# nirschl-lab/stain2stain

Hardware: AMD Instinct MI355X
Metric: paired 256x256 stain tiles/sec (full CFM optimisation step) (higher is better)
Workload: dtype bf16

## Files before the change

### include/stain2stain_hip.h

```cpp
#ifndef STAIN2STAIN_HIP_H
#define STAIN2STAIN_HIP_H

#ifdef __cplusplus
extern "C" {
#endif

#define S2S_OK 0
#define S2S_ERR_SHAPE (-1)
#define S2S_ERR_ALIGN (-2)
#define S2S_ERR_DTYPE (-3)
#define S2S_ERR_LAUNCH (-4)
#define S2S_ERR_NULL (-5)

#define S2S_BF16 0
#define S2S_F32 1

int s2s_conv3x3_stat_blocks(int dtype, int B, int H, int W, int Cout);
int s2s_conv3x3_nhwc(int dtype, const void* x0, int ld0, int c0, const void* x1, int ld1, int c1,
                     const void* w_packed, const float* bias, void* y, int ldy, float* stat_part,
                     const float* ep_scale, const float* ep_shift, int relu, int B, int H, int W, int Cout,
                     void* stream);

int s2s_conv3x3_ksplit(int dtype, int B, int H, int W, int Cout, int cin);
int s2s_conv3x3_nhwc_k(int dtype, const void* x0, int ld0, int c0, const void* x1, int ld1, int c1,
                       const void* w_packed, const float* bias, void* y, int ldy, float* stat_part,
                       const float* ep_scale, const float* ep_shift, int relu, float* kwork, int B, int H, int W,
                       int Cout, void* stream);
int s2s_conv3x3_stat_rows(int dtype, int B, int H, int W, int Cout, int c0, int c1, int ld0, int ld1, int has_bias);
int s2s_conv3x3_staged(int dtype, int B, int H, int W, int Cout, int c0, int c1, int ld0, int ld1, int ldy, int stats);
int s2s_conv3x3_family(int dtype, int B, int H, int W, int Cout, int c0, int c1, int ld0, int ld1, int ldy, int has_bias,
                       int has_affine, int stats, int stat_rows, int kwork);
int s2s_conv3x3_nhwc_s(int dtype, const void* x0, int ld0, int c0, const void* x1, int ld1, int c1, const void* w_packed,
                       const float* bias, void* y, int ldy, float* stat_part, int stat_rows, const float* ep_scale,
                       const float* ep_shift, int relu, float* kwork, int B, int H, int W, int Cout, void* stream);
int s2s_debug_conv_clock(long* out_host, int n);

int s2s_conv3x3_wgrad_splits(int dtype, int B, int H, int W, int Cin, int Cout);
int s2s_conv3x3_wgrad_nhwc(int dtype, const void* dy, int lddy, int Cout, const void* x0, int ld0, int c0,
                           const void* x1, int ld1, int c1, float* part, float* grad_oihw, int accumulate,
                           int B, int H, int W, void* stream);
int s2s_conv3x3_wgrad_phase(int dtype, const void* dy, int lddy, int Cout, const void* x0, int ld0, int c0,
                            const void* x1, int ld1, int c1, float* part, float* grad_oihw, int accumulate,
                            int B, int H, int W, int phases, void* stream);

int s2s_stem_stat_blocks(int B, int H, int W);
int s2s_stem_conv3x3_fwd(int dtype, const float* x_nchw, const float* w_oihw, const float* bias, void* y, int ldy,
                         float* stat_part, int B, int H, int W, int Cin, int Cout, void* stream);
int s2s_stem_wgrad_blocks(int B, int H, int W);
int s2s_stem_conv3x3_wgrad(int dtype, const void* dy, int lddy, const float* x_nchw, float* part, float* dw_oihw,
                           float* dbias, int accumulate, int B, int H, int W, int Cin, int Cout, void* stream);
int s2s_head_conv1x1_fwd(int dtype, const void* x, int ldx, const float* w, const float* bias, float* y_nchw, int B,
                         int H, int W, int C, int Cout, void* stream);
int s2s_head_wgrad_blocks(int B, int H, int W);
int s2s_head_conv1x1_bwd(int dtype, const float* dy_nchw, const void* x, int ldx, const float* w, void* dx, int lddx,
                         float* part, float* dw, float* dbias, int accumulate, int B, int H, int W, int C, int Cout,
                         void* stream);

int s2s_head_loss_blocks(int B, int H, int W);
int s2s_head_loss_fused(int dtype, const void* x, int ldx, const float* w, const float* bias, const float* u_nchw,
                        float* v_nchw, void* dx, int lddx, float grad_scale, float* part, double* lpart, float* dw,
                        float* dbias, float* loss, int accumulate, int B, int H, int W, int C, int Cout, void* stream);

int s2s_tail_blocks(int B, int H, int W);
int s2s_tail_fwd_loss(int dtype, const void* raw, int ldx, const float* scale, const float* shift, const float* mean,
                      const float* invstd, const float* w, const float* bias, const float* u_nchw, float* v_nchw,
                      float* g_nchw, float grad_scale, float* part, double* lpart, float* bnwork, float* dw,
                      float* dbias, float* loss, float* dgamma, float* dbeta, float* conv_dbias, int accumulate, int B,
                      int H, int W, int C, int Cout, void* stream);
int s2s_tail_bwd_apply(int dtype, const void* raw, int ldx, const float* g_nchw, const float* w, const float* scale,
                       const float* shift, const float* mean, const float* invstd, const float* gamma,
                       const float* bnwork, void* dx, int lddx, int B, int H, int W, int C, int Cout, void* stream);

int s2s_bn_finalize(const float* part, int nblk, int C, long count, const float* gamma, const float* beta,
                    float* running_mean, float* running_var, long* num_batches_tracked, float momentum, float eps,
                    float* mean, float* invstd, float* scale, float* shift, void* stream);
int s2s_bn_finalize_b(const float* part, int nblk, int C, long count, const float* gamma, const float* beta,
                      float* running_mean, float* running_var, long* num_batches_tracked, float momentum, float eps,
                      float* mean, float* invstd, float* scale, float* shift, const float* conv_bias, void* stream);
int s2s_bn_eval_prepare(int C, const float* gamma, const float* beta, const float* running_mean,
                        const float* running_var, float eps, float* scale, float* shift, void* stream);
int s2s_bn_relu_apply(int dtype, const void* x, int ldx, const float* scale, const float* shift, void* y, int ldy,
                      void* pool, int ldp, int B, int H, int W, int C, void* stream);
int s2s_maxpool2(int dtype, const void* x, int ldx, void* pool, int ldp, int B, int H, int W, int C, void* stream);
int s2s_bn_bwd_blocks(int B, int H, int W, int C);
int s2s_bn_relu_bwd(int dtype, const void* g1, int ldg1, const void* gp, int ldgp, const float* scale,
                    const float* shift, const void* x, int ldx, const float* mean, const float* invstd, const float* gamma, float* dgamma,
                    float* dbeta, float* dbias_conv, int accumulate, void* dx, int lddx, float* work, int B, int H,
                    int W, int C, void* stream);
int s2s_bn_partial_sums(const float* part, int nblk, int C, float* sums, void* stream);
int s2s_bn_relu_bwd_phase(int dtype, const void* g1, int ldg1, const void* gp, int ldgp, const float* scale,
                          const float* shift, const void* x, int ldx, const float* mean, const float* invstd,
                          const float* gamma, float* dgamma, float* dbeta, float* dbias_conv, int accumulate, void* dx,
                          int lddx, float* work, int B, int H, int W, int C, long count_total, int phases, void* stream);

int s2s_upsample2x_bilinear_ac_fwd(int dtype, const void* x, int ldx, const float* bias_nc, void* y, int ldy, int B,
                                   int Hin, int Win, int Hout, int Wout, int C, void* stream);
int s2s_upsample2x_bilinear_ac_bwd(int dtype, const void* dy, int lddy, void* dx, int lddx, int B, int Hin, int Win,
                                   int Hout, int Wout, int C, void* stream);
int s2s_upsample2x_bilinear_ac_bwd_ref(int dtype, const void* dy, int lddy, void* dx, int lddx, int B, int Hin,
                                       int Win, int Hout, int Wout, int C, void* stream);
int s2s_upsample2x_bwd_family(int lddy, int lddx, int B, int Hin, int Win, int Hout, int Wout, int C, int reference);
int s2s_pixel_sum(int dtype, const void* x, int ldx, float* out_nc, int B, int HW, int C, int accumulate,
                  void* stream);

int s2s_time_embedding(const float* t, float* out, int B, int dim, void* stream);
int s2s_linear_fwd(const float* x, const float* w, const float* bias, float* y, int B, int K, int N, void* stream);
int s2s_linear_bwd(const float* dy, const float* x, const float* w, float* dx, float* dw, float* db, int accumulate,
                   int B, int K, int N, void* stream);
int s2s_silu_fwd(const float* h, float* a, int n, void* stream);
int s2s_silu_bwd(const float* h, const float* da, float* dh, int n, void* stream);
int s2s_cfm_sample(const float* x0, const float* x1, const float* t, const float* eps, float sigma, float* xt,
                   float* ut, int B, long per_sample, void* stream);
int s2s_mse_loss(const float* v, const float* u, float* dv, float grad_scale, float* loss, double* work, long count,
                 void* stream);
int s2s_ode_error_norm(const float* e, const float* y0, const float* y1, float atol, float rtol, float* out,
                       double* work, long n, void* stream);
int s2s_axpy(float* x, const float* y, float a, long n, void* stream);
int s2s_dp_partials(long n);
int s2s_dp_init(int phase, const float* y, const float* k1, const float* fa, double* state, double* part, float* out,
                float* t_out, int* status, float atol, float rtol, int B, long n, void* stream);
int s2s_dp_stage(int i, const float* y, const float* k1, const float* k2, const float* k3, const float* k4,
                 const float* k5, const float* k6, const double* state, float* out, float* t_out, int B, long n,
                 void* stream);
int s2s_dp_error(const float* k1, const float* k2, const float* k3, const float* k4, const float* k5, const float* k6,
                 const float* k7, const float* y, const float* y_new, const double* state, double* part, float atol,
                 float rtol, int B, long n, void* stream);
int s2s_dp_control(double* state, const double* part, int* status, int max_steps, int B, long n, void* stream);
int s2s_dp_commit(float* y, const float* y_new, float* k1, const float* k7, const double* state, int B, long n,
                  void* stream);
int s2s_rk_stage(const float* x, const float* k1, const float* k2, const float* k3, float c1, float c2, float c3, int nk,
                 float* out, float* t_out, const float* table, const int* counter, int stages, int stage, int table_len,
                 int B, long n, void* stream);
int s2s_rk_combine(float* x, const float* k1, const float* k2, const float* k3, const float* k4, float c1, float c2,
                   float c3, float c4, int nk, int* counter, int B, long n, void* stream);
int s2s_fill_f32(float* x, float v, long n, void* stream);
int s2s_euler_tick(float* t, int n, const float* table, int* counter, void* stream);

int s2s_adam_step(float* p, const float* g, float* m, float* v, long n, int step, float lr, float beta1, float beta2,
                  float eps, float weight_decay, float grad_scale, void* stream);
int s2s_adam_step_dev(float* p, const float* g, float* m, float* v, long n, const float* hyper, void* stream);
long s2s_adam_multi_blocks(long n);
int s2s_adam_multi(const void* desc, int ntensors, long total, int step, float lr, float beta1, float beta2, float eps,
                   float weight_decay, float grad_scale, void* stream);
int s2s_adam_ema_step(float* p, const float* g, float* m, float* v, float* ema, long n, int step, float lr, float beta1,
                      float beta2, float eps, float weight_decay, float grad_scale, float ema_weight, void* stream);
int s2s_adam_ema_step_dev(float* p, const float* g, float* m, float* v, float* ema, long n, const float* hyper,
                          const float* ema_weight, void* stream);
long s2s_ema_multi_blocks(long n);
int s2s_ema_multi(const void* desc, int ntensors, long total, const float* weight, void* stream);
long s2s_pack_conv3x3_fwd_elems(int Cout, int Cin);
long s2s_pack_conv3x3_dgrad_elems(int Cout, int Cin);
int s2s_pack_conv3x3(int dtype, const float* w_oihw, void* w_fwd, void* w_dgrad, int Cout, int Cin, void* stream);
int s2s_pack_conv3x3_batched(int dtype, const void* desc, int nlayers, long total, void* stream);
int s2s_nchw_to_nhwc(int dtype, const float* x_nchw, void* y, int ldy, int B, int C, int H, int W, void* stream);
int s2s_nhwc_to_nchw(int dtype, const void* x, int ldx, float* y_nchw, int accumulate, int B, int C, int H, int W,
                     void* stream);

int s2s_paired_crop_flip_normalize(const void* src_u8, const void* tgt_u8, const int* params, float* out_src,
                                   float* out_tgt, int B, int Hs, int Ws, int S, void* stream);
int s2s_pil_resize_bilinear_normalize(const void* src_u8, void* tmp_u8, const int* bounds_h, const int* kk_h,
                                      int ksize_h, const int* bounds_v, const int* kk_v, int ksize_v, void* out_u8,
                                      float* out_f, int B, int Hs, int Ws, int Ho, int Wo, void* stream);

int s2s_region_gather(const void* img_u8, long pitch, int H, int W, int band_top, int band_h, const int* origins,
                      float* out, int B, int T, void* stream);
int s2s_region_blend(const float* tiles, int c0, const float* tiles1, int c1, const int* origins, int n, int T,
                     int overlap, float* acc, int band_rows, int H, int W, int r0, int r1, void* stream);
int s2s_region_finalize(float* acc, int band_rows, int W, int C, int r0, int r1, void* out_u8, long pitch_u8,
                        float* out_f, long pitch_f, int out_top, void* stream);

int s2s_region_tissue_count(const void* img_u8, long pitch, int H, int W, int band_top, int band_h, const int* origins,
                            int n, int T, int white, int black, int* counts, void* stream);
int s2s_region_skip_weight(const int* origins, int n, int T, int overlap, float* ws, int band_rows, int H, int W,
                           int r0, int r1, void* stream);
int s2s_region_finalize_mixed(float* acc, float* ws, int band_rows, int W, int C, int r0, int r1, const void* src_u8,
                              long src_pitch, int src_top, void* out_u8, long pitch_u8, float* out_f, long pitch_f,
                              int out_top, void* stream);

int s2s_seg_loss(const float* z, const float* g, float* dz, float* out, double* work, long n, float smooth,
// ... 175 lines not shown
```

### stain2stain_amd/csrc/resample.hip

```cpp
#include "common.h"
#include <stdlib.h>

namespace {

struct Axis {
  int i0, i1;
  float w0, w1;
};

__device__ __forceinline__ Axis ac_axis(int dst, int n_in, float scale) {
  Axis a;
  const float src = scale * (float)dst;
  a.i0 = (int)src;
  if (a.i0 > n_in - 1) a.i0 = n_in - 1;
  a.i1 = a.i0 + (a.i0 < n_in - 1 ? 1 : 0);
  a.w1 = src - (float)a.i0;
  a.w0 = 1.f - a.w1;
  return a;
}

__device__ __forceinline__ int rs_pcb(int C) {
  int p = 1;
  while (p < 32 && p * 8 < C) p <<= 1;
  return p;
}

template <typename T, bool BIAS>
__global__ __launch_bounds__(256) void upsample2x_fwd_kernel(const T* __restrict__ x, int ldx,
                                                             const float* __restrict__ bias, T* __restrict__ y,
                                                             int ldy, int B, int Hin, int Win, int Hout, int Wout,
                                                             int padT, int padL, int C, int band) {
  const int cp = C >> 3;
  const int Hu = 2 * Hin, Wu = 2 * Win;
  const float sh = Hu > 1 ? (float)(Hin - 1) / (float)(Hu - 1) : 0.f;
  const float sw = Wu > 1 ? (float)(Win - 1) / (float)(Wu - 1) : 0.f;
  const int PCB = rs_pcb(C), WL = 256 / PCB;
  const int pc = threadIdx.x & (PCB - 1), slot = threadIdx.x / PCB;
  const int nrows = B * Hout;
  for (int row0 = blockIdx.x * band; row0 < nrows; row0 += gridDim.x * band)
  for (int row = row0; row < row0 + band && row < nrows; ++row) {
    const int n = row / Hout, oy = row - n * Hout;
    const int uy = oy - padT;
    const bool row_in = uy >= 0 && uy < Hu;
    const Axis ay = ac_axis(row_in ? uy : 0, Hin, sh);
    const T* const r0 = x + ((long)n * Hin + ay.i0) * Win * ldx;
    const T* const r1 = x + ((long)n * Hin + ay.i1) * Win * ldx;
    T* const yr = y + (long)row * Wout * ldy;
    for (int pb = 0; pb < cp; pb += PCB) {
      const int c8 = (pb + pc) * 8;
      if (pb + pc >= cp) continue;
      float bv[8];
#pragma unroll
      for (int k = 0; k < 8; ++k) bv[k] = BIAS ? bias[(long)n * C + c8 + k] : 0.f;
      for (int ox = slot; ox < Wout; ox += WL) {
        const int ux = ox - padL;
        f32x8 o;
        if (!row_in || ux < 0 || ux >= Wu) {
#pragma unroll
          for (int k = 0; k < 8; ++k) o.v[k] = 0.f;
        } else {
          const Axis ax = ac_axis(ux, Win, sw);
          const int o0 = ax.i0 * ldx + c8, o1 = ax.i1 * ldx + c8;
          const f32x8 v00 = load8(r0 + o0), v01 = load8(r0 + o1), v10 = load8(r1 + o0), v11 = load8(r1 + o1);
#pragma unroll
          for (int k = 0; k < 8; ++k) {
            const float b = bv[k];
            o.v[k] = ay.w0 * (ax.w0 * (v00.v[k] + b) + ax.w1 * (v01.v[k] + b)) +
                     ay.w1 * (ax.w0 * (v10.v[k] + b) + ax.w1 * (v11.v[k] + b));
          }
        }
        store8(yr + ox * ldy + c8, o);
      }
    }
  }
}

template <typename T>
__global__ void upsample2x_bwd_kernel(const T* __restrict__ dy, int lddy, T* __restrict__ dx, int lddx, int B,
                                      int Hin, int Win, int Hout, int Wout, int padT, int padL, int C) {
  const int cp = C >> 3;
  const int Hu = 2 * Hin, Wu = 2 * Win;
  const float sh = Hu > 1 ? (float)(Hin - 1) / (float)(Hu - 1) : 0.f;
  const float sw = Wu > 1 ? (float)(Win - 1) / (float)(Wu - 1) : 0.f;
  const int total = B * Hin * Win * cp;
  for (int i = blockIdx.x * blockDim.x + threadIdx.x; i < total; i += gridDim.x * blockDim.x) {
    const int t0 = i / cp, c8 = (i - t0 * cp) * 8;
    const int t1 = t0 / Win, ix = t0 - t1 * Win;
    const int n = t1 / Hin, iy = t1 - n * Hin;
    int y_lo, y_hi, x_lo, x_hi;
    if (Hin == 1) { y_lo = 0; y_hi = Hu - 1; }
    else {
      y_lo = (int)floorf((float)(iy - 1) / sh) - 1; y_hi = (int)ceilf((float)(iy + 1) / sh) + 1;
      if (y_lo < 0) y_lo = 0;
      if (y_hi > Hu - 1) y_hi = Hu - 1;
    }
    if (Win == 1) { x_lo = 0; x_hi = Wu - 1; }
    else {
      x_lo = (int)floorf((float)(ix - 1) / sw) - 1; x_hi = (int)ceilf((float)(ix + 1) / sw) + 1;
      if (x_lo < 0) x_lo = 0;
      if (x_hi > Wu - 1) x_hi = Wu - 1;
    }
    constexpr int NSLOT = 12;
    float wxs[NSLOT];
#pragma unroll
    for (int j = 0; j < NSLOT; ++j) {
      const int ux = x_lo + j;
      float wx = 0.f;
      if (ux <= x_hi) {
        const Axis ax = ac_axis(ux, Win, sw);
        if (ax.i0 == ix) wx += ax.w0;
        if (ax.i1 == ix) wx += ax.w1;
        const int ox = ux + padL;
        if (ox < 0 || ox >= Wout) wx = 0.f;
      }
      wxs[j] = wx;
    }
    f32x8 acc;
#pragma unroll
    for (int k = 0; k < 8; ++k) acc.v[k] = 0.f;
    for (int uy = y_lo; uy <= y_hi; ++uy) {
      const Axis ay = ac_axis(uy, Hin, sh);
      float wy = 0.f;
      if (ay.i0 == iy) wy += ay.w0;
      if (ay.i1 == iy) wy += ay.w1;
      const int oy = uy + padT;
      if (wy == 0.f || oy < 0 || oy >= Hout) continue;
      const T* const rowp = dy + (((long)n * Hout + oy) * Wout + x_lo + padL) * lddy + c8;
#pragma unroll
      for (int j = 0; j < NSLOT; ++j) {
        if (wxs[j] == 0.f) continue;
        const f32x8 g = load8(rowp + (long)j * lddy);
        const float w = wy * wxs[j];
#pragma unroll
        for (int k = 0; k < 8; ++k) acc.v[k] += w * g.v[k];
      }
    }
    store8(dx + (((long)n * Hin + iy) * Win + ix) * lddx + c8, acc);
  }
}

__device__ __forceinline__ float ac_weight_of(int dst, int n_in, float scale, int src_index) {
  const Axis a = ac_axis(dst, n_in, scale);
  return (a.i0 == src_index ? a.w0 : 0.f) + (a.i1 == src_index ? a.w1 : 0.f);
}

template <typename T>
__global__ void upsample2x_bwd_win_kernel(const T* __restrict__ dy, int lddy, T* __restrict__ dx, int lddx, int B,
                                          int Hin, int Win, int Hout, int Wout, int padT, int padL, int C) {
  const int cp = C >> 3;
  const int Hu = 2 * Hin, Wu = 2 * Win;
  const float sh = (float)(Hin - 1) / (float)(Hu - 1), sw = (float)(Win - 1) / (float)(Wu - 1);
  const int total = B * Hin * Win * cp;
  for (int i = blockIdx.x * blockDim.x + threadIdx.x; i < total; i += gridDim.x * blockDim.x) {
    const int t0 = i / cp, c8 = (i - t0 * cp) * 8;
// ... 122 lines not shown
      Raw8<T> cur[6];
#pragma unroll
      for (int m = 0; m < 6; ++m) cur[m] = load_raw8(rowp[j] + off[m]);
      f32x8 g[6];
#pragma unroll
      for (int m = 0; m < 6; ++m) g[m] = widen8(cur[m]);
      if (j < 4) {
#pragma unroll
        for (int m = 0; m < 4; ++m) {
          const float w = wyA[j] * wxA[m];
#pragma unroll
          for (int k = 0; k < 8; ++k) a00.v[k] = fmaf(w, g[m].v[k], a00.v[k]);
        }
#pragma unroll
        for (int m = 0; m < 4; ++m) {
          const float w = wyA[j] * wxB[m];
#pragma unroll
          for (int k = 0; k < 8; ++k) a01.v[k] = fmaf(w, g[m + 2].v[k], a01.v[k]);
        }
      }
      if (j >= 2) {
#pragma unroll
        for (int m = 0; m < 4; ++m) {
          const float w = wyB[j - 2] * wxA[m];
#pragma unroll
          for (int k = 0; k < 8; ++k) a10.v[k] = fmaf(w, g[m].v[k], a10.v[k]);
        }
#pragma unroll
        for (int m = 0; m < 4; ++m) {
          const float w = wyB[j - 2] * wxB[m];
#pragma unroll
          for (int k = 0; k < 8; ++k) a11.v[k] = fmaf(w, g[m + 2].v[k], a11.v[k]);
        }
      }
      if (j < 4) { pin8(a00); pin8(a01); }
      if (j >= 2) { pin8(a10); pin8(a11); }
      __builtin_amdgcn_sched_barrier(0);
    }
    store8(dr0 + ix0 * lddx, a00);
    store8(dr0 + (ix0 + 1) * lddx, a01);
    store8(dr1 + ix0 * lddx, a10);
    store8(dr1 + (ix0 + 1) * lddx, a11);
  }
}

template <typename T>
__global__ void pixel_sum_kernel(const T* __restrict__ x, int ldx, float* __restrict__ out, int HW, int C,
                                 int accumulate) {
  const int n = blockIdx.y;
  const int c = blockIdx.x * 64 + (threadIdx.x & 63);
  const int rg = threadIdx.x >> 6;
  float s = 0.f;
  if (c < C) {
    constexpr int U = 16;
    const T* const xp = x + (long)n * HW * ldx + c;
    int p = rg;
    for (; p + 4 * (U - 1) < HW; p += 4 * U) {
      float v[U];
#pragma unroll
      for (int u = 0; u < U; ++u) v[u] = to_f32(xp[(long)(p + 4 * u) * ldx]);
#pragma unroll
      for (int u = 0; u < U; ++u) s += v[u];
    }
    for (; p < HW; p += 4) s += to_f32(xp[(long)p * ldx]);
  }
  __shared__ float red[4][64];
  red[rg][threadIdx.x & 63] = s;
  __syncthreads();
  if (rg == 0 && c < C) {
    s = red[0][threadIdx.x] + red[1][threadIdx.x] + red[2][threadIdx.x] + red[3][threadIdx.x];
    out[(long)n * C + c] = accumulate ? out[(long)n * C + c] + s : s;
  }
}

inline int ew_grid(long total) {
  long b = (total + 255) / 256;
  if (b > 8192) b = 8192;
  if (b < 1) b = 1;
  return (int)b;
}

}

extern "C" int s2s_upsample2x_bilinear_ac_fwd(int dtype, const void* x, int ldx, const float* bias_nc, void* y,
                                              int ldy, int B, int Hin, int Win, int Hout, int Wout, int C,
                                              void* stream) {
  if (!x || !y) return S2S_ERR_NULL;
  if (B <= 0 || Hin <= 0 || Win <= 0 || C <= 0 || (C % 8) || (ldx % 8) || (ldy % 8)) return S2S_ERR_SHAPE;
  if (Hout < 2 * Hin || Wout < 2 * Win) return S2S_ERR_SHAPE;
  const int padT = (Hout - 2 * Hin) / 2, padL = (Wout - 2 * Win) / 2;
  if ((long)Win * ldx >= (1L << 31) || (long)Wout * ldy >= (1L << 31) || (long)B * Hout >= (1L << 31))
    return S2S_ERR_SHAPE;
  hipStream_t s = (hipStream_t)stream;
  const long rows = (long)B * Hout;
  static const int band_env = [] { const char* e = getenv("S2S_UP_BAND"); return e ? atoi(e) : 0; }();
  const int band = band_env > 0 ? band_env : (rows >= 4096 ? 4 : rows >= 2048 ? 2 : 1);
  const long nwg = (rows + band - 1) / band;
  const dim3 grid((unsigned)(nwg < 65535 * 4 ? nwg : 65535 * 4));
#define S2S_UP(TT, BB)                                                                                          \
  hipLaunchKernelGGL((upsample2x_fwd_kernel<TT, BB>), grid, dim3(256), 0, s, (const TT*)x, ldx, bias_nc, (TT*)y, \
                     ldy, B, Hin, Win, Hout, Wout, padT, padL, C, band)
  if (dtype == S2S_BF16) { if (bias_nc) S2S_UP(bf16_t, true); else S2S_UP(bf16_t, false); }
  else if (dtype == S2S_F32) { if (bias_nc) S2S_UP(float, true); else S2S_UP(float, false); }
  else return S2S_ERR_DTYPE;
#undef S2S_UP
  S2S_LAUNCH_CHECK();
  return S2S_OK;
}

namespace {

enum UpBwdFamily { kUpBwdGather = 0, kUpBwdWindow = 1, kUpBwdQuad = 2 };

int upsample2x_bwd_family(int lddy, int lddx, int B, int Hin, int Win, int Wout, int C, bool reference) {
  if (!(Hin > 3 && Win > 3)) return kUpBwdGather;
  const long nwork = (long)B * ((Hin + 1) / 2);
  const bool quad = !reference && Hin <= 4096 && Win <= 4096 && (long)Wout * lddy < (1L << 31) &&
                    (long)Win * lddx < (1L << 31) && nwork * cdiv(C / 8, 32) < (1L << 31);
  return quad ? kUpBwdQuad : kUpBwdWindow;
}

int upsample2x_bwd_launch(int dtype, const void* dy, int lddy, void* dx, int lddx, int B, int Hin, int Win, int Hout,
                          int Wout, int C, void* stream, bool reference) {
  if (!dy || !dx) return S2S_ERR_NULL;
  if (B <= 0 || Hin <= 0 || Win <= 0 || C <= 0 || (C % 8) || (lddy % 8) || (lddx % 8)) return S2S_ERR_SHAPE;
  if (Hout < 2 * Hin || Wout < 2 * Win) return S2S_ERR_SHAPE;
  const int padT = (Hout - 2 * Hin) / 2, padL = (Wout - 2 * Win) / 2;
  const long total = (long)B * Hin * Win * (C / 8);
  if (total >= (1L << 31) - (1L << 22)) return S2S_ERR_SHAPE;
  hipStream_t s = (hipStream_t)stream;
  const dim3 grid(ew_grid(total));
  if (dtype != S2S_BF16 && dtype != S2S_F32) return S2S_ERR_DTYPE;
  const int family = upsample2x_bwd_family(lddy, lddx, B, Hin, Win, Wout, C, reference);
  const bool win = family != kUpBwdGather;
  const int nchunk = cdiv(C / 8, 32);
  const long nwork = (long)B * ((Hin + 1) / 2);
  if (family == kUpBwdQuad) {
    const dim3 qgrid((unsigned)(nwork * nchunk));
    if (dtype == S2S_BF16)
      hipLaunchKernelGGL(upsample2x_bwd_quad_kernel<bf16_t>, qgrid, dim3(256), 0, s, (const bf16_t*)dy, lddy,
                         (bf16_t*)dx, lddx, B, Hin, Win, Hout, Wout, padT, padL, C, (int)nwork);
    else
      hipLaunchKernelGGL(upsample2x_bwd_quad_kernel<float>, qgrid, dim3(256), 0, s, (const float*)dy, lddy, (float*)dx,
                         lddx, B, Hin, Win, Hout, Wout, padT, padL, C, (int)nwork);
    S2S_LAUNCH_CHECK();
    return S2S_OK;
  }
#define S2S_UPB(KERN, TT)                                                                                           \
  hipLaunchKernelGGL(KERN<TT>, grid, dim3(256), 0, s, (const TT*)dy, lddy, (TT*)dx, lddx, B, Hin, Win, Hout, Wout,   \
                     padT, padL, C)
  if (dtype == S2S_BF16) { if (win) S2S_UPB(upsample2x_bwd_win_kernel, bf16_t); else S2S_UPB(upsample2x_bwd_kernel, bf16_t); }
  else { if (win) S2S_UPB(upsample2x_bwd_win_kernel, float); else S2S_UPB(upsample2x_bwd_kernel, float); }
#undef S2S_UPB
  S2S_LAUNCH_CHECK();
  return S2S_OK;
}

}

extern "C" int s2s_upsample2x_bilinear_ac_bwd(int dtype, const void* dy, int lddy, void* dx, int lddx, int B, int Hin,
                                              int Win, int Hout, int Wout, int C, void* stream) {
  return upsample2x_bwd_launch(dtype, dy, lddy, dx, lddx, B, Hin, Win, Hout, Wout, C, stream, false);
}

extern "C" int s2s_upsample2x_bilinear_ac_bwd_ref(int dtype, const void* dy, int lddy, void* dx, int lddx, int B,
                                                  int Hin, int Win, int Hout, int Wout, int C, void* stream) {
  return upsample2x_bwd_launch(dtype, dy, lddy, dx, lddx, B, Hin, Win, Hout, Wout, C, stream, true);
}

extern "C" int s2s_upsample2x_bwd_family(int lddy, int lddx, int B, int Hin, int Win, int Hout, int Wout, int C,
                                         int reference) {
  if (B <= 0 || Hin <= 0 || Win <= 0 || C <= 0 || (C % 8) || (lddy % 8) || (lddx % 8)) return S2S_ERR_SHAPE;
  if (Hout < 2 * Hin || Wout < 2 * Win) return S2S_ERR_SHAPE;
  if ((long)B * Hin * Win * (C / 8) >= (1L << 31) - (1L << 22)) return S2S_ERR_SHAPE;
  return upsample2x_bwd_family(lddy, lddx, B, Hin, Win, Wout, C, reference != 0);
}

extern "C" int s2s_pixel_sum(int dtype, const void* x, int ldx, float* out_nc, int B, int HW, int C, int accumulate,
                             void* stream) {
  if (!x || !out_nc) return S2S_ERR_NULL;
  if (B <= 0 || HW <= 0 || C <= 0) return S2S_ERR_SHAPE;
  hipStream_t s = (hipStream_t)stream;
  dim3 grid(cdiv(C, 64), B);
  if (dtype == S2S_BF16)
    hipLaunchKernelGGL(pixel_sum_kernel<bf16_t>, grid, dim3(256), 0, s, (const bf16_t*)x, ldx, out_nc, HW, C, accumulate);
  else if (dtype == S2S_F32)
    hipLaunchKernelGGL(pixel_sum_kernel<float>, grid, dim3(256), 0, s, (const float*)x, ldx, out_nc, HW, C, accumulate);
  else return S2S_ERR_DTYPE;
  S2S_LAUNCH_CHECK();
  return S2S_OK;
// ... 2 lines not shown
```

### stain2stain_amd/ops.py

```python
from __future__ import annotations

import contextlib
import ctypes
import os
import sys
from typing import Optional, Tuple

import torch

from . import _native

BF16, F32 = 0, 1


def _dt(t: torch.Tensor) -> int:
    if t.dtype == torch.bfloat16:
        return BF16
    if t.dtype == torch.float32:
        return F32
    raise RuntimeError(f"stain2stain_amd: unsupported activation dtype {t.dtype}")


_raw_stream = getattr(torch._C, "_cuda_getCurrentRawStream", None)
_raw_device = getattr(torch._C, "_cuda_getDevice", None)
# ... 427 lines not shown
                                _f32(running_var), 0 if num_batches is None else num_batches.data_ptr(), momentum, eps,
                                out[0].data_ptr(), out[1].data_ptr(), out[2].data_ptr(), out[3].data_ptr(),
                                _f32(conv_bias), _stream())
    _native.check(rc, "bn_finalize")
    return out


def bn_partial_sums(stat: torch.Tensor) -> torch.Tensor:
    _, C, nblk = stat.shape
    sums = torch.empty((2, C), dtype=torch.float32, device=stat.device)
    _native.check(_L().s2s_bn_partial_sums(_f32(stat), nblk, C, _f32(sums), _stream()), "bn_partial_sums")
    return sums


def bn_eval_prepare(gamma, beta, rmean, rvar, eps: float = 1e-5):
    C = gamma.numel()
    out = torch.empty((2, C), dtype=torch.float32, device=gamma.device)
    rc = _L().s2s_bn_eval_prepare(C, _f32(gamma), _f32(beta), _f32(rmean), _f32(rvar), eps, out[0].data_ptr(),
                                  out[1].data_ptr(), _stream())
    _native.check(rc, "bn_eval_prepare")
    return out


@_timed("bn_relu_apply")
def bn_relu_apply(x: torch.Tensor, scale: torch.Tensor, shift: torch.Tensor, out: Optional[torch.Tensor] = None,
                  pool: Optional[torch.Tensor] = None, want_pool: bool = False):
    B, H, W, C = x.shape
    px, ldx = _nhwc(x)
    if out is None:
        out = torch.empty((B, H, W, C), dtype=x.dtype, device=x.device)
    py, ldy = _nhwc(out)
    pp, ldp = 0, 8
    if want_pool and pool is None:
        pool = torch.empty((B, H // 2, W // 2, C), dtype=x.dtype, device=x.device)
    if pool is not None:
        pp, ldp = _nhwc(pool)
    rc = _L().s2s_bn_relu_apply(_dt(x), px, ldx, _f32(scale), _f32(shift), py, ldy, pp, ldp, B, H, W, C, _stream())
    _native.check(rc, "bn_relu_apply")
    return out, pool


@_timed("maxpool2")
def maxpool2(x: torch.Tensor) -> torch.Tensor:
    B, H, W, C = x.shape
    px, ldx = _nhwc(x)
    pool = torch.empty((B, H // 2, W // 2, C), dtype=x.dtype, device=x.device)
    rc = _L().s2s_maxpool2(_dt(x), px, ldx, pool.data_ptr(), C, B, H, W, C, _stream())
    _native.check(rc, "maxpool2")
    return pool


@_timed("bn_relu_bwd")
def bn_relu_bwd(g1: Optional[torch.Tensor], gp: Optional[torch.Tensor], x: torch.Tensor,
                stats: torch.Tensor, gamma: torch.Tensor, dgamma: torch.Tensor, dbeta: torch.Tensor,
                dbias_conv: Optional[torch.Tensor], accumulate: bool = False, exchange=None,
                count_total: Optional[int] = None) -> torch.Tensor:
    B, H, W, C = x.shape
    px, ldx = _nhwc(x)
    p1, ld1 = (0, 8) if g1 is None else _nhwc(g1)
    p2, ld2 = (0, 8) if gp is None else _nhwc(gp)
    dx = torch.empty((B, H, W, C), dtype=x.dtype, device=x.device)
    nb = _L().s2s_bn_bwd_blocks(B, H, W, C)
    work = torch.empty((4 * nb * C + 2 * C,), dtype=torch.float32, device=x.device)
    if exchange is not None:
        for phase in (1, 2):
            rc = _L().s2s_bn_relu_bwd_phase(_dt(x), p1, ld1, p2, ld2, stats[2].data_ptr(), stats[3].data_ptr(), px, ldx,
                                            stats[0].data_ptr(), stats[1].data_ptr(),
                                            _f32(gamma), _f32(dgamma), _f32(dbeta), _f32(dbias_conv), int(accumulate),
                                            dx.data_ptr(), C, _f32(work), B, H, W, C,
                                            int(count_total if count_total is not None else B * H * W), phase, _stream())
            _native.check(rc, "bn_relu_bwd")
            if phase == 1:
                exchange(work[4 * nb * C:])
        return dx
    rc = _L().s2s_bn_relu_bwd(_dt(x), p1, ld1, p2, ld2, stats[2].data_ptr(), stats[3].data_ptr(), px, ldx,
                              stats[0].data_ptr(), stats[1].data_ptr(),
                              _f32(gamma), _f32(dgamma), _f32(dbeta), _f32(dbias_conv), int(accumulate),
                              dx.data_ptr(), C, _f32(work), B, H, W, C, _stream())
    _native.check(rc, "bn_relu_bwd")
    return dx


@_timed("upsample2x_fwd")
def upsample2x_fwd(x: torch.Tensor, out: torch.Tensor, bias_nc: Optional[torch.Tensor] = None) -> None:
    B, Hin, Win, C = x.shape
    _, Hout, Wout, Co = out.shape
    if Co != C or out.dtype != x.dtype:
        raise RuntimeError("stain2stain_amd: upsample output slice mismatch")
    px, ldx = _nhwc(x)
    py, ldy = _nhwc(out)
    rc = _L().s2s_upsample2x_bilinear_ac_fwd(_dt(x), px, ldx, _f32(bias_nc), py, ldy, B, Hin, Win, Hout, Wout, C,
                                             _stream())
    _native.check(rc, "upsample2x_fwd")


@_timed("upsample2x_bwd")
def upsample2x_bwd(dy: torch.Tensor, hin: int, win: int, _reference: bool = False) -> torch.Tensor:
    B, Hout, Wout, C = dy.shape
    pdy, lddy = _nhwc(dy)
    dx = torch.empty((B, hin, win, C), dtype=dy.dtype, device=dy.device)
    fn = _L().s2s_upsample2x_bilinear_ac_bwd_ref if _reference else _L().s2s_upsample2x_bilinear_ac_bwd
    rc = fn(_dt(dy), pdy, lddy, dx.data_ptr(), C, B, hin, win, Hout, Wout, C, _stream())
    _native.check(rc, "upsample2x_bwd")
    return dx


def upsample2x_bwd_family(dy: torch.Tensor, hin: int, win: int, _reference: bool = False) -> int:
    B, Hout, Wout, C = dy.shape
    rc = _L().s2s_upsample2x_bwd_family(dy.stride(2), C, B, hin, win, Hout, Wout, C, int(_reference))
    if rc < 0:
        _native.check(rc, "upsample2x_bwd_family")
    return rc


def pixel_sum(x: torch.Tensor) -> torch.Tensor:
    B, H, W, C = x.shape
    px, ldx = _nhwc(x)
    out = torch.empty((B, C), dtype=torch.float32, device=x.device)
    rc = _L().s2s_pixel_sum(_dt(x), px, ldx, _f32(out), B, H * W, C, 0, _stream())
    _native.check(rc, "pixel_sum")
    return out


def time_embedding(t: torch.Tensor, dim: int) -> torch.Tensor:
    t = t.reshape(-1).to(torch.float32).contiguous()
    out = torch.empty((t.numel(), dim), dtype=torch.float32, device=t.device)
    _native.check(_L().s2s_time_embedding(_f32(t), _f32(out), t.numel(), dim, _stream()), "time_embedding")
    return out


def linear_fwd(x: torch.Tensor, w: torch.Tensor, b: Optional[torch.Tensor]) -> torch.Tensor:
    B, K = x.shape
    N = w.shape[0]
    y = torch.empty((B, N), dtype=torch.float32, device=x.device)
    _native.check(_L().s2s_linear_fwd(_f32(x), _f32(w), _f32(b), _f32(y), B, K, N, _stream()), "linear_fwd")
    return y


def linear_bwd(dy: torch.Tensor, x: torch.Tensor, w: torch.Tensor, dw: torch.Tensor, db: Optional[torch.Tensor],
               need_dx: bool = True, accumulate: bool = False) -> Optional[torch.Tensor]:
    B, K = x.shape
    N = w.shape[0]
    dx = torch.empty((B, K), dtype=torch.float32, device=x.device) if need_dx else None
    _native.check(_L().s2s_linear_bwd(_f32(dy), _f32(x), _f32(w), _f32(dx), _f32(dw), _f32(db), int(accumulate), B, K,
                                      N, _stream()), "linear_bwd")
    return dx


def silu_fwd(h: torch.Tensor) -> torch.Tensor:
    a = torch.empty_like(h)
    _native.check(_L().s2s_silu_fwd(_f32(h), _f32(a), h.numel(), _stream()), "silu_fwd")
    return a


def silu_bwd(h: torch.Tensor, da: torch.Tensor) -> torch.Tensor:
    dh = torch.empty_like(h)
    _native.check(_L().s2s_silu_bwd(_f32(h), _f32(da), _f32(dh), h.numel(), _stream()), "silu_bwd")
    return dh


@_timed("cfm_sample")
def cfm_sample(x0: torch.Tensor, x1: torch.Tensor, t: torch.Tensor, sigma: float = 0.0,
               eps: Optional[torch.Tensor] = None):
    xt = torch.empty_like(x0)
    ut = torch.empty_like(x0)
    B = x0.shape[0]
    _native.check(_L().s2s_cfm_sample(_f32(x0), _f32(x1), _f32(t), _f32(eps), float(sigma), _f32(xt), _f32(ut), B,
                                      x0.numel() // B, _stream()), "cfm_sample")
    return xt, ut


@_timed("mse_loss")
def mse_loss(v: torch.Tensor, u: torch.Tensor, want_grad: bool = True, grad_scale: float = 1.0):
    loss = torch.empty((), dtype=torch.float32, device=v.device)
    dv = torch.empty_like(v) if want_grad else None
    work = torch.empty((1024,), dtype=torch.float64, device=v.device)
# ... 1182 lines not shown
```

Measured before the change: 2255.

## Add source-row-centric upsample2x forward kernel reusing each 2x2 input quad

Adds an upsample forward kernel where each workgroup owns one input row and channel chunk. Each thread loads the four neighbouring input vectors once and writes every output pixel whose interpolation base is that input pixel, instead of reloading four inputs per output pixel. It is used for the unpadded exact-2x case. The blend is rewritten with explicit FMAs and contraction disabled so the new kernel matches the per-pixel kernel bit for bit. A reference entry point and a family query are added so the old path can still be selected for testing.

Measured after the change: 2288 (median of 6 runs). Within noise of the previous version (+1.5%).

```diff
diff --git a/include/stain2stain_hip.h b/include/stain2stain_hip.h
--- a/include/stain2stain_hip.h
+++ b/include/stain2stain_hip.h
@@ -95,6 +95,9 @@
 
 int s2s_upsample2x_bilinear_ac_fwd(int dtype, const void* x, int ldx, const float* bias_nc, void* y, int ldy, int B,
                                    int Hin, int Win, int Hout, int Wout, int C, void* stream);
+int s2s_upsample2x_bilinear_ac_fwd_ref(int dtype, const void* x, int ldx, const float* bias_nc, void* y, int ldy, int B,
+                                       int Hin, int Win, int Hout, int Wout, int C, void* stream);
+int s2s_upsample2x_fwd_family(int ldx, int ldy, int B, int Hin, int Win, int Hout, int Wout, int C, int reference);
 int s2s_upsample2x_bilinear_ac_bwd(int dtype, const void* dy, int lddy, void* dx, int lddx, int B, int Hin, int Win,
                                    int Hout, int Wout, int C, void* stream);
 int s2s_upsample2x_bilinear_ac_bwd_ref(int dtype, const void* dy, int lddy, void* dx, int lddx, int B, int Hin,
diff --git a/stain2stain_amd/csrc/resample.hip b/stain2stain_amd/csrc/resample.hip
--- a/stain2stain_amd/csrc/resample.hip
+++ b/stain2stain_amd/csrc/resample.hip
@@ -23,6 +23,37 @@
   int p = 1;
   while (p < 32 && p * 8 < C) p <<= 1;
   return p;
+}
+
+__device__ __forceinline__ Axis ac_axis_fwd(int dst, int n_in, float scale) {
+#pragma clang fp contract(off)
+  Axis a;
+  const float d = (float)dst;
+  a.i0 = (int)(scale * d);
+  if (a.i0 > n_in - 1) a.i0 = n_in - 1;
+  a.i1 = a.i0 + (a.i0 < n_in - 1 ? 1 : 0);
+  a.w1 = __builtin_fmaf(scale, d, -(float)a.i0);
+  a.w0 = 1.f - a.w1;
+  return a;
+}
+
+__device__ __forceinline__ f32x8 up_blend8(const Axis& ay, const Axis& ax, const f32x8& v00, const f32x8& v01,
+                                           const f32x8& v10, const f32x8& v11, const float* bv) {
+#pragma clang fp contract(off)
+  f32x8 o;
+#pragma unroll
+  for (int k = 0; k < 8; ++k) {
+    const float b = bv[k];
+    const float a00 = v00.v[k] + b, a01 = v01.v[k] + b, a10 = v10.v[k] + b, a11 = v11.v[k] + b;
+    if (k & 1) {
+      const float top = __builtin_fmaf(ax.w0, a00, ax.w1 * a01), bot = __builtin_fmaf(ax.w0, a10, ax.w1 * a11);
+      o.v[k] = __builtin_fmaf(ay.w0, top, ay.w1 * bot);
+    } else {
+      const float top = __builtin_fmaf(ax.w1, a01, ax.w0 * a00), bot = __builtin_fmaf(ax.w1, a11, ax.w0 * a10);
+      o.v[k] = __builtin_fmaf(ay.w1, bot, ay.w0 * top);
+    }
+  }
+  return o;
 }
 
 template <typename T, bool BIAS>
@@ -42,7 +73,7 @@
     const int n = row / Hout, oy = row - n * Hout;
     const int uy = oy - padT;
     const bool row_in = uy >= 0 && uy < Hu;
-    const Axis ay = ac_axis(row_in ? uy : 0, Hin, sh);
+    const Axis ay = ac_axis_fwd(row_in ? uy : 0, Hin, sh);
     const T* const r0 = x + ((long)n * Hin + ay.i0) * Win * ldx;
     const T* const r1 = x + ((long)n * Hin + ay.i1) * Win * ldx;
     T* const yr = y + (long)row * Wout * ldy;
@@ -59,17 +90,60 @@
 #pragma unroll
           for (int k = 0; k < 8; ++k) o.v[k] = 0.f;
         } else {
-          const Axis ax = ac_axis(ux, Win, sw);
+          const Axis ax = ac_axis_fwd(ux, Win, sw);
           const int o0 = ax.i0 * ldx + c8, o1 = ax.i1 * ldx + c8;
           const f32x8 v00 = load8(r0 + o0), v01 = load8(r0 + o1), v10 = load8(r1 + o0), v11 = load8(r1 + o1);
-#pragma unroll
-          for (int k = 0; k < 8; ++k) {
-            const float b = bv[k];
-            o.v[k] = ay.w0 * (ax.w0 * (v00.v[k] + b) + ax.w1 * (v01.v[k] + b)) +
-                     ay.w1 * (ax.w0 * (v10.v[k] + b) + ax.w1 * (v11.v[k] + b));
-          }
+          o = up_blend8(ay, ax, v00, v01, v10, v11, bv);
         }
         store8(yr + ox * ldy + c8, o);
+      }
+    }
+  }
+}
+
+template <typename T, bool BIAS>
+__global__ __launch_bounds__(256, 4) void upsample2x_fwd_rows_kernel(const T* __restrict__ x, int ldx,
+                                                                     const float* __restrict__ bias,
+                                                                     T* __restrict__ y, int ldy, int B, int Hin,
+                                                                     int Win, int C, int nwork) {
+  const int cp = C >> 3;
+  const int Hu = 2 * Hin, Wu = 2 * Win;
+  const float sh = (float)(Hin - 1) / (float)(Hu - 1), sw = (float)(Win - 1) / (float)(Wu - 1);
+  const int PCB = rs_pcb(C), WL = 256 / PCB;
+  const int pc = threadIdx.x & (PCB - 1), slot = threadIdx.x / PCB;
+  const int nwg = gridDim.x, q = nwg >> 3, r = nwg & 7, cls = blockIdx.x & 7;
+  const int wgid = (cls < r ? cls * (q + 1) : r * (q + 1) + (cls - r) * q) + (blockIdx.x >> 3);
+  const int chunk = wgid / nwork, work = wgid - chunk * nwork;
+  const int n = work / Hin, i = work - n * Hin;
+  const int piece = chunk * PCB + pc;
+  if (piece >= cp) return;
+  const int c8 = piece * 8;
+
+  Axis ay[3];
+  bool own_y[3];
+#pragma unroll
+  for (int a = 0; a < 3; ++a) {
+    const int oy = 2 * i + a;
+    ay[a] = ac_axis_fwd(oy, Hin, sh);
+    own_y[a] = oy < Hu && ay[a].i0 == i;
+  }
+  const T* const r0 = x + ((long)n * Hin + i) * Win * ldx + c8;
+  const T* const r1 = x + ((long)n * Hin + i + (i < Hin - 1 ? 1 : 0)) * Win * ldx + c8;
+  T* const yr = y + ((long)n * Hu + 2 * i) * Wu * ldy + c8;
+  float bv[8];
+#pragma unroll
+  for (int k = 0; k < 8; ++k) bv[k] = BIAS ? bias[(long)n * C + c8 + k] : 0.f;
+  for (int j = slot; j < Win; j += WL) {
+    const int o0 = j * ldx, o1 = (j + (j < Win - 1 ? 1 : 0)) * ldx;
+    const f32x8 v00 = load8(r0 + o0), v01 = load8(r0 + o1), v10 = load8(r1 + o0), v11 = load8(r1 + o1);
+#pragma unroll
+    for (int m = 0; m < 3; ++m) {
+      const int ox = 2 * j + m;
+      const Axis ax = ac_axis_fwd(ox, Win, sw);
+      if (ox < Wu && ax.i0 == j) {
+#pragma unroll
+        for (int a = 0; a < 3; ++a)
+          if (own_y[a]) store8(yr + ((long)a * Wu + ox) * ldy, up_blend8(ay[a], ax, v00, v01, v10, v11, bv));
       }
     }
   }
@@ -358,30 +432,75 @@
 
 }
 
-extern "C" int s2s_upsample2x_bilinear_ac_fwd(int dtype, const void* x, int ldx, const float* bias_nc, void* y,
-                                              int ldy, int B, int Hin, int Win, int Hout, int Wout, int C,
-                                              void* stream) {
-  if (!x || !y) return S2S_ERR_NULL;
+namespace {
+
+enum UpFwdFamily { kUpFwdPixel = 0, kUpFwdRows = 1 };
+
+int upsample2x_fwd_shape_error(int ldx, int ldy, int B, int Hin, int Win, int Hout, int Wout, int C) {
   if (B <= 0 || Hin <= 0 || Win <= 0 || C <= 0 || (C % 8) || (ldx % 8) || (ldy % 8)) return S2S_ERR_SHAPE;
   if (Hout < 2 * Hin || Wout < 2 * Win) return S2S_ERR_SHAPE;
-  const int padT = (Hout - 2 * Hin) / 2, padL = (Wout - 2 * Win) / 2;
   if ((long)Win * ldx >= (1L << 31) || (long)Wout * ldy >= (1L << 31) || (long)B * Hout >= (1L << 31))
     return S2S_ERR_SHAPE;
+  return S2S_OK;
+}
+
+int upsample2x_fwd_family(int B, int Hin, int Win, int Hout, int Wout, int C, bool reference) {
+  const bool rows = !reference && Hout == 2 * Hin && Wout == 2 * Win && Hin >= 2 && Win >= 2 && Hin <= 4096 &&
+                    Win <= 4096 && (long)B * Hin * cdiv(C / 8, 32) < (1L << 31);
+  return rows ? kUpFwdRows : kUpFwdPixel;
+}
+
+int upsample2x_fwd_launch(int dtype, const void* x, int ldx, const float* bias_nc, void* y, int ldy, int B, int Hin,
+                          int Win, int Hout, int Wout, int C, void* stream, bool reference) {
+  if (!x || !y) return S2S_ERR_NULL;
+  const int err = upsample2x_fwd_shape_error(ldx, ldy, B, Hin, Win, Hout, Wout, C);
+  if (err != S2S_OK) return err;
+  if (dtype != S2S_BF16 && dtype != S2S_F32) return S2S_ERR_DTYPE;
+  const int padT = (Hout - 2 * Hin) / 2, padL = (Wout - 2 * Win) / 2;
   hipStream_t s = (hipStream_t)stream;
+  const bool rowsk = upsample2x_fwd_family(B, Hin, Win, Hout, Wout, C, reference) == kUpFwdRows;
   const long rows = (long)B * Hout;
   static const int band_env = [] { const char* e = getenv("S2S_UP_BAND"); return e ? atoi(e) : 0; }();
   const int band = band_env > 0 ? band_env : (rows >= 4096 ? 4 : rows >= 2048 ? 2 : 1);
   const long nwg = (rows + band - 1) / band;
   const dim3 grid((unsigned)(nwg < 65535 * 4 ? nwg : 65535 * 4));
-#define S2S_UP(TT, BB)                                                                                          \
-  hipLaunchKernelGGL((upsample2x_fwd_kernel<TT, BB>), grid, dim3(256), 0, s, (const TT*)x, ldx, bias_nc, (TT*)y, \
-                     ldy, B, Hin, Win, Hout, Wout, padT, padL, C, band)
+  const int nwork = B * Hin;
+  const dim3 rgrid((unsigned)((long)nwork * cdiv(C / 8, 32)));
+#define S2S_UP(TT, BB)                                                                                            \
+  do {                                                                                                            \
+    if (rowsk)                                                                                                    \
+      hipLaunchKernelGGL((upsample2x_fwd_rows_kernel<TT, BB>), rgrid, dim3(256), 0, s, (const TT*)x, ldx, bias_nc, \
+                         (TT*)y, ldy, B, Hin, Win, C, nwork);                                                     \
+    else                                                                                                          \
+      hipLaunchKernelGGL((upsample2x_fwd_kernel<TT, BB>), grid, dim3(256), 0, s, (const TT*)x, ldx, bias_nc,       \
+                         (TT*)y, ldy, B, Hin, Win, Hout, Wout, padT, padL, C, band);                              \
+  } while (0)
   if (dtype == S2S_BF16) { if (bias_nc) S2S_UP(bf16_t, true); else S2S_UP(bf16_t, false); }
-  else if (dtype == S2S_F32) { if (bias_nc) S2S_UP(float, true); else S2S_UP(float, false); }
-  else return S2S_ERR_DTYPE;
+  else { if (bias_nc) S2S_UP(float, true); else S2S_UP(float, false); }
 #undef S2S_UP
   S2S_LAUNCH_CHECK();
   return S2S_OK;
+}
+
+}
+
+extern "C" int s2s_upsample2x_bilinear_ac_fwd(int dtype, const void* x, int ldx, const float* bias_nc, void* y,
+                                              int ldy, int B, int Hin, int Win, int Hout, int Wout, int C,
+                                              void* stream) {
+  return upsample2x_fwd_launch(dtype, x, ldx, bias_nc, y, ldy, B, Hin, Win, Hout, Wout, C, stream, false);
+}
+
+extern "C" int s2s_upsample2x_bilinear_ac_fwd_ref(int dtype, const void* x, int ldx, const float* bias_nc, void* y,
+                                                  int ldy, int B, int Hin, int Win, int Hout, int Wout, int C,
+                                                  void* stream) {
+  return upsample2x_fwd_launch(dtype, x, ldx, bias_nc, y, ldy, B, Hin, Win, Hout, Wout, C, stream, true);
+}
+
+extern "C" int s2s_upsample2x_fwd_family(int ldx, int ldy, int B, int Hin, int Win, int Hout, int Wout, int C,
+                                         int reference) {
+  const int err = upsample2x_fwd_shape_error(ldx, ldy, B, Hin, Win, Hout, Wout, C);
+  if (err != S2S_OK) return err;
+  return upsample2x_fwd_family(B, Hin, Win, Hout, Wout, C, reference != 0);
 }
 
 namespace {
diff --git a/stain2stain_amd/ops.py b/stain2stain_amd/ops.py
--- a/stain2stain_amd/ops.py
+++ b/stain2stain_amd/ops.py
@@ -533,16 +533,26 @@
 
 
 @_timed("upsample2x_fwd")
-def upsample2x_fwd(x: torch.Tensor, out: torch.Tensor, bias_nc: Optional[torch.Tensor] = None) -> None:
+def upsample2x_fwd(x: torch.Tensor, out: torch.Tensor, bias_nc: Optional[torch.Tensor] = None,
+                   _reference: bool = False) -> None:
     B, Hin, Win, C = x.shape
     _, Hout, Wout, Co = out.shape
     if Co != C or out.dtype != x.dtype:
         raise RuntimeError("stain2stain_amd: upsample output slice mismatch")
     px, ldx = _nhwc(x)
     py, ldy = _nhwc(out)
-    rc = _L().s2s_upsample2x_bilinear_ac_fwd(_dt(x), px, ldx, _f32(bias_nc), py, ldy, B, Hin, Win, Hout, Wout, C,
-                                             _stream())
+    fn = _L().s2s_upsample2x_bilinear_ac_fwd_ref if _reference else _L().s2s_upsample2x_bilinear_ac_fwd
+    rc = fn(_dt(x), px, ldx, _f32(bias_nc), py, ldy, B, Hin, Win, Hout, Wout, C, _stream())
     _native.check(rc, "upsample2x_fwd")
+
+
+def upsample2x_fwd_family(x: torch.Tensor, out: torch.Tensor, _reference: bool = False) -> int:
+    B, Hin, Win, C = x.shape
+    _, Hout, Wout, _ = out.shape
+    rc = _L().s2s_upsample2x_fwd_family(_nhwc(x)[1], _nhwc(out)[1], B, Hin, Win, Hout, Wout, C, int(_reference))
+    if rc < 0:
+        _native.check(rc, "upsample2x_fwd_family")
+    return rc
 
 
 @_timed("upsample2x_bwd")
```
